# bigpon/QPNet

Measured on AMD Instinct MI355X. Metric: train steps/sec (batch-1 chunk-steps of RF+20000 samples, aggregate over GPUs), higher is better.
Workload: dtype f32; 1 GPU; config[1]: paper-size SI-QPNet (C=64,S=256,4F+4A) training step, forward+CE+backward+Adam on one chunk of 20900 samples (RF 946 + batch_length 19954), batch 1 per GPU; global_batch=1, parallelism=dp1 (utterance-sharded chunks, one flat-gradient all-reduce per step), backend=none, world_size=1, aux_1x1=frame rate (hoisted: K = 128 + one 4-deep step)

## Files before the change

qpnet_amd/csrc/train_bwd.hip:

```cpp
#include "train_common.h"
#include "train_post.h"
#include "qpn_handle.h"
#include <string.h>
#include <stdlib.h>
#include <math.h>

template <int MT>
__global__ __launch_bounds__(512) void k_post_bwd(TrainParams p, TrainBwd bw) {
    constexpr int TM = 16 * MT;
    extern __shared__ float sm[];
    const int S = p.S, Q = p.Q, LC = p.LC;
    const int ldp = tr_lda(Q > S ? Q : S), ldr = tr_lda(S);
    float* P = sm; float* R = sm + TM * ldp;
    const int b = blockIdx.y, t0 = blockIdx.x * TM;
    const int tid = threadIdx.x, lane = tid & 63, wave = tid >> 6;
    const int NTS = S / 16;
    const int npairs = (NTS + 1) / 2;
    const int np0 = wave < npairs ? wave : 0;
    const int pnt[2] = {2 * np0, (2 * np0 + 1 < NTS) ? 2 * np0 + 1 : 2 * np0};
    float my[2][MT][4], ms[2][MT][4];
    auto mask_load = [&](const float* src, float (&m)[2][MT][4]) {
#pragma unroll
        for (int j = 0; j < 2; ++j)
#pragma unroll
// ... 932 lines not shown
            for (int l = 0; l < w.nlayers; ++l) { sub.goff[l] = w.goff[l] + m0 * w.ldc; if (w.gbias[l] >= 0) sub.gbias[l] = w.gbias[l] + m0; }
            sub.ncol_groups = wgrad_col_groups(sub.M, sub.N);
            ok = wgrad2_any(sub, nch, generic, stream);
        }
        return ok;
    }
    if (wgrad3_any(w, nch, generic, stream)) return true;
    switch (w.bmode) {
    case 4: return false;
    case 1: return wgrad2_mode<1>(w, nch, stream);
    case 2: return wgrad2_mode<2>(w, nch, stream);
    case 3: return wgrad2_mode<3>(w, nch, stream);
    default: return wgrad2_mode<0>(w, nch, stream);
    }
}

__global__ void k_reduce_grad_s(const float* __restrict__ slab, const int* __restrict__ gdst, const int* __restrict__ gdst_list, const int* __restrict__ gzero, int n_gzero,
                                int nch, int gstage, int64_t n, float* __restrict__ g, float scale, int append_scale, int s0, int s1, int skip0, int skip1, int tail,
                                const int* __restrict__ status, int flag_again) {
    int64_t i = (int64_t)blockIdx.x * blockDim.x + threadIdx.x + s0;
    if (flag_again && append_scale && i == s0) g[n + 1] = (status && *status) ? 1.f : 0.f;
    if (i < s1) {
        if (i >= skip0 && i < skip1) return;
        const int k0 = gdst[i], k1 = gdst[i + 1];
        if (k0 == k1) return;
        float a = 0.f;
        const float* sp = slab + i;
        int c = 0;
        for (; c + 8 <= nch; c += 8) {
            float v[8];
#pragma unroll
            for (int k = 0; k < 8; ++k) v[k] = sp[(size_t)(c + k) * gstage];
            a += ((v[0] + v[1]) + (v[2] + v[3])) + ((v[4] + v[5]) + (v[6] + v[7]));
        }
        for (; c < nch; ++c) a += sp[(size_t)c * gstage];
        a *= scale;
        for (int k = k0; k < k1; ++k) g[gdst_list[k]] = a;
        return;
    }
    if (!tail) return;
    const int64_t j = i - s1;
    if (j < n_gzero) g[gzero[j]] = 0.f;
    else if (append_scale && j < n_gzero + 4 && !(flag_again && j == n_gzero + 1)) g[n + (j - n_gzero)] = j == n_gzero ? scale : (j == n_gzero + 1 && status && *status) ? 1.f : 0.f;
}

__global__ __launch_bounds__(256) void k_causal_bwd(TrainParams p, TrainBwd bw, int rows_per_wg, int CB) {
    extern __shared__ float tab[];
    const int C = p.C, Q = p.Q;
    const int tid = threadIdx.x;
    const int64_t total = (int64_t)p.B * p.N1;
    const int64_t r0 = (int64_t)blockIdx.x * rows_per_wg, r1 = r0 + rows_per_wg < total ? r0 + rows_per_wg : total;
    for (int cb = 0; cb < C; cb += CB) {
        const int cbv = C - cb < CB ? C - cb : CB;
        for (int i = tid; i < 2 * Q * CB; i += 256) tab[i] = 0.f;
        __syncthreads();
        const int cpr = cbv;
        for (int64_t idx = r0 * cpr + tid; idx < r1 * cpr; idx += 256) {
            const int64_t rr = idx / cpr; const int c = (int)(idx - rr * cpr);
            const int b = (int)(rr / p.N1), n = (int)(rr - (int64_t)b * p.N1);
            const size_t o = ((size_t)b * p.N1 + n) * C + cb + c;
            const float v = bw.DXA[0][o] + bw.DXB[0][o];
            const int64_t xo = (int64_t)p.T - p.N0 + n;
            int64_t s0 = p.x[(size_t)b * p.T + xo] % Q, s1 = p.x[(size_t)b * p.T + xo + 1] % Q;
            if (s0 < 0) s0 += Q;
            if (s1 < 0) s1 += Q;
            atomicAdd(&tab[(0 * Q + s0) * CB + c], v);
            atomicAdd(&tab[(1 * Q + s1) * CB + c], v);
        }
        __syncthreads();
        for (int i = tid; i < 2 * Q * cbv; i += 256) {
            const int c = i / (2 * Q), qt = i - c * 2 * Q, q = qt >> 1, tp = qt & 1;
            const float v = tab[(tp * Q + q) * CB + c];
            if (v != 0.f) atomicAdd(&bw.gflat[p.causal_w + ((size_t)(cb + c) * Q + q) * 2 + tp], v * bw.gscale);
        }
        for (int c = tid; c < cbv; c += 256) {
            float s = 0.f;
            for (int q = 0; q < Q; ++q) s += tab[(0 * Q + q) * CB + c];
            atomicAdd(&bw.gflat[p.causal_b + cb + c], s * bw.gscale);
        }
        __syncthreads();
    }
}

__global__ __launch_bounds__(128) void k_up_bwd(UpArgs u) { up_bwd_body(u, blockIdx.x, blockIdx.y, threadIdx.x, 128); }

__global__ __launch_bounds__(128) void k_aux_tail(AuxArgs p) {
    __shared__ float hrow[1024];
    __shared__ float red[2];
    const AuxGeom& ag = p.g;
    const int C = p.C, A = p.A, L = p.L, tid = threadIdx.x;
    const int bx = blockIdx.x;
    float v = 0.f;
    const bool role_a = bx < L * A;
    if (role_a) {
        const int l = bx / A, a = bx - l * A, n = tid;
        const size_t wi = (n < C ? ag.auxS[l] + (size_t)n * A : ag.auxT[l] + (size_t)(n - C) * A) + a;
        const float va = p.flat[wi];
        float e = 0.f;
        {
            float ev[TR_EB_SLOTS];
#pragma unroll
            for (int k = 0; k < TR_EB_SLOTS; ++k) ev[k] = p.EB[(size_t)(l * TR_EB_SLOTS + k) * 2 * C + n];
#pragma unroll
            for (int k = 0; k < TR_EB_SLOTS; ++k) e += ev[k];
        }
        float acc = 0.f;
        for (int b = 0; b < p.B; ++b) {
            const float* hb = p.h + ((size_t)b * A + a) * p.F + p.ffirst;
            const float* D = p.DPA + (size_t)(l * p.B + b) * (p.nfr + 1) * 2 * C + n;
            for (int f0 = 0; f0 < p.nfr; f0 += 1024) {
                const int nf = p.nfr - f0 < 1024 ? p.nfr - f0 : 1024;
                __syncthreads();
                for (int i = tid; i < nf; i += 128) hrow[i] = hb[f0 + i];
                __syncthreads();
                int f = 0;
                for (; f + 64 <= nf; f += 64) {
                    float d[64];
#pragma unroll
                    for (int k = 0; k < 64; ++k) d[k] = D[(size_t)(f0 + f + k) * 2 * C];
#pragma unroll
                    for (int k = 0; k < 64; ++k) acc += d[k] * hrow[f + k];
                }
                for (; f + 16 <= nf; f += 16) {
                    float d[16];
#pragma unroll
                    for (int k = 0; k < 16; ++k) d[k] = D[(size_t)(f0 + f + k) * 2 * C];
#pragma unroll
                    for (int k = 0; k < 16; ++k) acc += d[k] * hrow[f + k];
                }
                for (; f < nf; ++f) acc += D[(size_t)(f0 + f) * 2 * C] * hrow[f];
            }
        }
        p.gflat[wi] = (acc + p.flat[p.up_b] * e) * p.gscale;
        v = va * e;
    } else {
        const int j = bx - L * A;
        const int q0 = p.F * p.U - p.N1;
        const int items = L * p.B * p.nfr;
        for (int it = tid; it < items; it += 128) {
            const int fx = it % p.nfr, lb = it / p.nfr, l = lb / p.B;
            const int n = (p.ffirst + fx) * p.U + j - q0;
            if (n >= ag.s_out[l] && n < p.N1) v += p.GW[(size_t)lb * p.N1 + n];
        }
    }
    for (int sft = 32; sft >= 1; sft >>= 1) v += __shfl_xor(v, sft);
    if ((tid & 63) == 0) red[tid >> 6] = v;
    __syncthreads();
    if (tid == 0) {
        if (role_a) atomicAdd(p.gflat + p.up_b, (red[0] + red[1]) * p.gscale);
        else p.gflat[p.up_w + (bx - L * A)] = (red[0] + red[1]) * p.gscale;
    }
}

struct AdamReports { int* h_status; double* h_loss; const double* d_loss; };
__device__ __forceinline__ float adam_update(float* __restrict__ w, float* __restrict__ m, float* __restrict__ v, int64_t i, float gi,
                                             float lr, float b1, float b2, float eps, float wd, float bc1, float bc2_sqrt) {
    if (wd != 0.f) gi += wd * w[i];
    const float mi = m[i] + (gi - m[i]) * (1.0f - b1);
    const float vi = v[i] * b2 + (1.0f - b2) * gi * gi;
    m[i] = mi; v[i] = vi;
    const float denom = sqrtf(vi) / bc2_sqrt + eps;
    const float wn = w[i] - (lr / bc1) * (mi / denom);
    w[i] = wn;
    return wn;
}
template <bool EMA>
// ... 278 lines not shown
            } else {
                ok = ok && wgrad2_any(w, nch_side_, gen, st);
                w.A = bw.DY0; w.lda = S; w.M = S; w.B1 = p.S0; w.goff[0] = sl.g_p1; w.gbias[0] = sl.g_bp1;
                ok = ok && wgrad2_any(w, nch_side_, gen, st);
            }
            qpn_prof_mark(PG_WGRAD_POST, st);
        }
    };
    auto build_w1 = [&]() {
        Wg2 w = wbase;
        w.A = bw.DZ; w.A2 = nullptr; w.A_lstride = (size_t)B * N1 * 2 * C; w.lda = 2 * C; w.M = 2 * C; w.rowsA = N1;
        w.bmode = 3; w.B1 = p.X; w.B2 = nullptr; w.B_lstride = nDX; w.ldb = C; w.N = p.Ktp; w.Nvalid = p.hoist ? 2 * C : 2 * C + p.Ap; w.rowsB = N1;
        w.nlayers = L; w.ldc = p.Ktp; w.ncol_groups = wgrad_col_groups(w.M, w.N);
        for (int l = 0; l < L; ++l) {
            const TrLayer& ly = p.layers[l];
            w.row0A[l] = w.row0B[l] = ly.s_out; w.R[l] = N1 - ly.s_out; w.goff[l] = sl.g_w1[l]; w.gbias[l] = sl.g_b1[l];
            w.tap_off[l] = ly.tap_off; w.dil[l] = ly.dilation;
        }
        return w;
    };
    auto build_wr = [&]() {
        Wg2 w = wbase;
        w.A = bw.DXA[0] + nDX; w.A2 = wr_summed ? nullptr : bw.DXB[0] + nDX; w.A_lstride = nDX; w.lda = C; w.M = C; w.rowsA = N1;
        w.bmode = 0; w.B1 = p.TH; w.B2 = nullptr; w.B_lstride = nDX; w.ldb = C; w.N = C; w.Nvalid = C; w.rowsB = N1; w.ldc = C;
        w.nlayers = L; w.ncol_groups = wgrad_col_groups(w.M, w.N);
        for (int l = 0; l < L; ++l) {
            w.row0A[l] = w.row0B[l] = p.layers[l].s_out;
            w.R[l] = l == L - 1 ? 0 : N1 - p.layers[l].s_out; w.goff[l] = sl.g_wr[l]; w.gbias[l] = sl.g_br[l]; w.tap_off[l] = -1; w.dil[l] = 0;
        }
        return w;
    };
    const bool early_reduce = overlap && bw.gdst && sl.g_early1 > sl.g_early0 && k.reduce_early;
    const bool up_side = early_reduce && p.U > 0 && k.up_side;
    if (early_reduce) {
        nch_side_ = k.wgrad_chunks_side > 0 && k.wgrad_chunks_side <= nch ? k.wgrad_chunks_side : (nch <= 48 ? nch : 48);
    }
    if (overlap) {
        QPN_HIP(hipEventRecord(ev_fork, stream));
        QPN_HIP(hipStreamWaitEvent(side, ev_fork, 0));
        qpn_prof_mark(-1, side);
        launch_skip_post(side);
        if (early_reduce) { launch_reduce_early(bw, side, up_side ? 1 : 0, nch_side_); qpn_prof_mark(PG_GRAD_TAIL, side); }
        if (early_reduce && up_side && bw.ev_early && bw.early_recorded) { QPN_HIP(hipEventRecord(bw.ev_early, side)); *bw.early_recorded = 1; }
    }
    const int swz = k.xcd_swizzle ? 1 : 0;
    if (p.hoist && !persist) { qpn_set_error("internal: the frame-rate aux term needs the register-resident layer kernels"); return QPN_EINVAL; }
    if (stack_q) {
        const int rcq = qpn_launch_stack_bwd(p, bw, *sq, k, stream);
        if (rcq) return rcq;
    }
    for (int l = L - 1; l >= 0 && !stack_q; --l) {
        const TrLayer& ly = p.layers[l];
        const int rows = N1 - ly.s_out;
        const int tiles = (rows + 15) / 16;
        if (persist) {
            int G = qpn_num_cus() * 2; if (G > tiles) G = tiles;
            if (G > 1024) G = 1024;
            const size_t ldsp = (size_t)(8 * 16 * tr_lda(C) + 16 * tr_lda(2 * C) + 16 * tr_lda(p.Ktp) + 64) * sizeof(float);
            const bool last = l == L - 1;
            const void* kf = p.hoist ? (last ? (const void*)k_layer_bwd_p<8, true> : (const void*)k_layer_bwd_p<8, false>)
                                     : (last ? (const void*)k_layer_bwd_p<11, true> : (const void*)k_layer_bwd_p<11, false>);
            (void)hipFuncSetAttribute(kf, hipFuncAttributeMaxDynamicSharedMemorySize, (int)ldsp);
            if (p.hoist) {
                if (last) hipLaunchKernelGGL((k_layer_bwd_p<8, true>), dim3(G, B), dim3(256), ldsp, stream, p, bw, l, swz ? 2 : 0, tiles, p.scratch_rows);
                else hipLaunchKernelGGL((k_layer_bwd_p<8, false>), dim3(G, B), dim3(256), ldsp, stream, p, bw, l, swz ? 2 : 0, tiles, p.scratch_rows);
            } else {
                if (last) hipLaunchKernelGGL((k_layer_bwd_p<11, true>), dim3(G, B), dim3(256), ldsp, stream, p, bw, l, swz ? 2 : 0, tiles, p.scratch_rows);
                else hipLaunchKernelGGL((k_layer_bwd_p<11, false>), dim3(G, B), dim3(256), ldsp, stream, p, bw, l, swz ? 2 : 0, tiles, p.scratch_rows);
            }
        } else {
            if (lds_layer > 48 * 1024) (void)hipFuncSetAttribute((const void*)k_layer_bwd<1>, hipFuncAttributeMaxDynamicSharedMemorySize, (int)lds_layer);
            hipLaunchKernelGGL((k_layer_bwd<1>), dim3(tiles, B), dim3(256), lds_layer, stream, p, bw, l, l == L - 1 ? 1 : 0, swz);
        }
    }
    auto build_causal = [&]() {
        Wg2 w = wbase;
        w.nlayers = 2; w.ncol_groups = Q / (Q % 64 == 0 ? 64 : 128);      w.bmode = 4; w.xc = p.XC; w.B1 = w.B2 = nullptr; w.B_lstride = 0;
        w.A = bw.DXA[0]; w.A2 = bw.DXB[0]; w.A_lstride = 0; w.lda = C; w.M = C; w.rowsA = N1;
        w.N = Q; w.Nvalid = Q; w.rowsB = N1 + 1; w.ldb = 0; w.ldc = Q;
        for (int tp = 0; tp < 2; ++tp) { w.row0A[tp] = 0; w.row0B[tp] = tp; w.R[tp] = N1; w.goff[tp] = sl.g_cw + tp * C * Q; w.gbias[tp] = tp == 0 ? sl.g_cb : -1; w.tap_off[tp] = -1; w.dil[tp] = 0; }
        return w;
    };
    const bool wr_side = overlap && k.wr_side;
    if (wr_side || up_side) {
        QPN_HIP(hipEventRecord(bw.ev_mid, stream));
        QPN_HIP(hipStreamWaitEvent(side, bw.ev_mid, 0));
        qpn_prof_mark(-1, side);
        if (up_side) { if (p.hoist) launch_aux_tail(p, bw, ag, side); else launch_up_bwd(p, bw, side); qpn_prof_mark(PG_GRAD_TAIL, side); }
        if (wr_side) { ok = ok && wgrad2_any(build_wr(), nch, gen, side); qpn_prof_mark(PG_WGRAD_WR, side); }
    }
    if (overlap) QPN_HIP(hipEventRecord(ev_join, side));
    qpn_prof_mark(PG_LAYER_BWD, stream);
    ok = ok && wgrad2_any(build_w1(), nch, gen, stream);
    qpn_prof_mark(PG_WGRAD, stream);
    if (!wr_side) { ok = ok && wgrad2_any(build_wr(), nch, gen, stream); qpn_prof_mark(PG_WGRAD_WR, stream); }
    if (!overlap) launch_skip_post(stream);
    if (sl.g_cw >= 0) ok = ok && wgrad2_any(build_causal(), nch, gen, stream);
    qpn_prof_mark(PG_WGRAD_CAUSAL, stream);
    if (overlap) { QPN_HIP(hipStreamWaitEvent(stream, ev_join, 0)); qpn_prof_mark(-1, stream); }
    if (!ok) { qpn_set_error("weight-gradient tiles: unsupported geometry (n_resch <= 128 on this path; wider stacks take the GEMM path)"); return QPN_EINVAL; }
    return qpn_launch_grad_tail(p, bw, &ag, stream, early_reduce, up_side);
}

int qpn_launch_adam(float* w, const float* g, float* m, float* v, int64_t n, int step, float lr, float b1, float b2, float eps, float wd, const float* den, int* status,
                    int* h_status, double* h_loss, const double* d_loss, float* e, float omd, hipStream_t stream) {
    const double bc1 = 1.0 - pow((double)b1, step), bc2 = 1.0 - pow((double)b2, step);
    AdamReports rep; rep.h_status = status ? h_status : nullptr; rep.h_loss = d_loss ? h_loss : nullptr; rep.d_loss = d_loss;
    if (e) hipLaunchKernelGGL(k_adam_ema, dim3((unsigned)((n + 255) / 256)), dim3(256), 0, stream, w, g, m, v, n, lr, b1, b2, eps, wd, (float)bc1, (float)sqrt(bc2), den, status, rep, e, omd);
    else hipLaunchKernelGGL(k_adam, dim3((unsigned)((n + 255) / 256)), dim3(256), 0, stream, w, g, m, v, n, lr, b1, b2, eps, wd, (float)bc1, (float)sqrt(bc2), den, status, rep);
    qpn_prof_mark(PG_ADAM, stream);
    QPN_HIP(hipGetLastError());
    return QPN_OK;
}

int qpn_launch_adam_clip(float* w, const float* g, float* m, float* v, int64_t n, int step, float lr, float b1, float b2, float eps, float wd, const float* den, int* status,
                         int* h_status, double* h_loss, const double* d_loss, float max_norm, double* part, double* d_norm, double* h_norm, float* e, float omd, hipStream_t stream) {
    const double bc1 = 1.0 - pow((double)b1, step), bc2 = 1.0 - pow((double)b2, step);
    AdamReports rep; rep.h_status = status ? h_status : nullptr; rep.h_loss = d_loss ? h_loss : nullptr; rep.d_loss = d_loss;
    const int64_t want = ((n >> 2) + 1 + 255) / 256;
    const int nb = want < TR_GN_BLOCKS ? (int)want : TR_GN_BLOCKS;
    hipLaunchKernelGGL(k_grad_sumsq, dim3(nb), dim3(256), 0, stream, g, n, part);
    if (e) hipLaunchKernelGGL(k_adam_clip_ema, dim3((unsigned)((n + 255) / 256)), dim3(256), 0, stream, w, g, m, v, n, lr, b1, b2, eps, wd, (float)bc1, (float)sqrt(bc2), den, status, rep,
                              (const double*)part, nb, max_norm, d_norm, h_norm, e, omd);
    else hipLaunchKernelGGL(k_adam_clip, dim3((unsigned)((n + 255) / 256)), dim3(256), 0, stream, w, g, m, v, n, lr, b1, b2, eps, wd, (float)bc1, (float)sqrt(bc2), den, status, rep,
                            (const double*)part, nb, max_norm, d_norm, h_norm);
    qpn_prof_mark(PG_ADAM, stream);
    QPN_HIP(hipGetLastError());
    return QPN_OK;
}

int qpn_launch_grad_accum(float* acc, const float* g, int64_t cnt, int first, const int* status, int* h_status, double* h_loss, const double* d_loss, hipStream_t stream) {
    AdamReports rep; rep.h_status = status ? h_status : nullptr; rep.h_loss = d_loss ? h_loss : nullptr; rep.d_loss = d_loss;
    const int64_t want = ((cnt >> 2) + 1 + 255) / 256, cap = (int64_t)qpn_num_cus() * 8;
    const int nb = (int)(want < cap ? want : cap);
    hipLaunchKernelGGL(k_grad_accum, dim3(nb), dim3(256), 0, stream, acc, g, cnt, first ? 1 : 0, status, rep);
    qpn_prof_mark(PG_ADAM, stream);
    QPN_HIP(hipGetLastError());
    return QPN_OK;
}
```

qpnet_amd/csrc/train_common.h:

```cpp
#pragma once
#include "qpn_common.h"

typedef float f32x4 __attribute__((ext_vector_type(4)));

#define TR_MAXL QPN_MAX_LAYERS

__host__ __device__ static inline int tr_lda(int K) { return ((K + 29) / 32) * 32 + 2; }
__host__ __device__ static inline int tr_ldt(int N) { return ((N + 15) / 32) * 32 + 16; }

struct TrLayer {
    int adaptive, dilation;
    int s_in, s_out;
    int tap_off;
    int w1_f4, wr_f4;
    int w1t_f4, wrt_f4;
    int bias1, biasr;
};

struct TrainParams {
    int C, S, Q, A, Ap, L, U;
    int B, T, F, Td, BL, N1, N0, maxd;
    int Kt, Ktp;
    int LC;
    const float* flat;
// ... 6 lines not shown
    float* HUP;
    int hoist;
    int nfr, ffirst;
    float* PA;
    float2* WJ;
    int* TAP;
    int* XC;
    float* S0; float* Y0;
    float* logits;
    const int64_t* ce_tgt; int64_t ce_stride; float* ce_dlogits; double* ce_loss;
    int* status;
    float* scratch_rows;
    unsigned* qctl;
    int4* qtab;
    int4* qtab_b;
    int qtotal;
    int qP[TR_MAXL + 1];
    int qT[TR_MAXL];
    int ws_f4, p1_f4, p2_f4;
    int wst_f4, p1t_f4, p2t_f4;
    int bias_s, bias_p1, bias_p2;
    int64_t causal_w, causal_b, up_w, up_b;
    TrLayer layers[TR_MAXL];
};

struct TrainSlabs {
    int g_w1[TR_MAXL], g_b1[TR_MAXL], g_wr[TR_MAXL], g_br[TR_MAXL], g_ws[TR_MAXL], g_bs;
    int g_p1, g_bp1, g_p2, g_bp2;
    int g_early0, g_early1;
    int g_cw, g_cb;
};

struct TrainBwd {
    const float* dlogits; float* gflat;
    float* DXA[2]; float* DXB[2];
    float* DZ;
    float* DS0; float* DY0;
    float* DGS;
    float* DHUP;
    float* DPA;
    float* GW;
    float* EB;
    float* slab;
    const int* gdst; const int* gdst_list;
    const int* gzero; int n_gzero;
    int nch, gstage;
    int64_t n_params;
    const struct TrainSlabs* sl;
    float gscale;
    int append_scale;
    const int* status;
    hipStream_t side; hipEvent_t ev_fork, ev_join, ev_mid;
    hipEvent_t ev_early; int* early_recorded;
};


struct AuxGeom { int auxS[TR_MAXL], auxT[TR_MAXL], bias1[TR_MAXL], s_out[TR_MAXL]; };
struct AuxArgs {
    const float* flat; const float* h; float* PA; float* bp; const float* DPA; const float* EB; const float* GW; float* gflat;
    float gscale; int C, A, L, B, F, U, N1, nfr, ffirst; int64_t up_w, up_b;
    AuxGeom g;
};
static inline AuxArgs tr_aux_args(const TrainParams& p, const TrainBwd* bw, const AuxGeom& ag) {
    AuxArgs a; a.flat = p.flat; a.h = p.h; a.PA = p.PA; a.bp = p.bp; a.DPA = bw ? bw->DPA : nullptr; a.EB = bw ? bw->EB : nullptr; a.GW = bw ? bw->GW : nullptr;
    a.gflat = bw ? bw->gflat : nullptr; a.gscale = bw ? bw->gscale : 1.f;
    a.C = p.C; a.A = p.A; a.L = p.L; a.B = p.B; a.F = p.F; a.U = p.U; a.N1 = p.N1; a.nfr = p.nfr; a.ffirst = p.ffirst; a.up_w = p.up_w; a.up_b = p.up_b; a.g = ag;
    return a;
}
struct RefreshArgs { const int* wmap; float* wout; int64_t nw; const int* bstart; const int* blist; int nb; double* loss; };
struct TrainKnobs {
    bool serial;
    bool stack_q_fwd, stack_q_bwd;
    int stack_wgs, stack_wgs_bwd;
    bool persist_fwd, persist_bwd;
    bool wgrad_generic;
    int wgrad_chunks, wgrad_chunks_side;
    bool post_fuse;
    bool up_side, reduce_early, wr_side;
    bool post_pair, zero_in_post, post_wide;
    bool xcd_swizzle;
    bool ce_separate;
    bool event_fence;
    bool prep_fuse;
    bool aux_hoist;
    bool test_stack_gives_up;
};
void qpn_train_knobs_parse(TrainKnobs& k);

#define TR_QHEAD_STRIDE 1056
#define TR_QHDR_WORDS 17920
struct StackQ {
    unsigned* flags;
    unsigned* head;
    unsigned* stats;
    unsigned* abort;
    const int4* tab;
    unsigned epoch;
    unsigned epoch_pub;
    unsigned spin_limit;
    int total, nq;
};

__host__ __device__ __forceinline__ int tr_pa_off(const TrainParams& p, int l, int b, int n0) {
    const int q = p.F * p.U - p.N1 + n0;
    return ((l * p.B + b) * (p.nfr + 1) + (q / p.U - p.ffirst)) * 2 * p.C;
}

__device__ __forceinline__ void tr_queue_entry_fwd(const TrainParams& p, int pos, int4& a, int4& b) {
    const bool valid = pos < p.qtotal;
    const int ps = valid ? pos : 0;
    int l = 0;
    for (int k = 1; k < p.L; ++k) l += ps >= p.qP[k] ? 1 : 0;
    const int r = ps - p.qP[l], T = p.qT[l];
    const int bi = r / T, t = r - bi * T;
    const TrLayer ly = p.layers[l];
    const int n0 = ly.s_out + 16 * t;
    int first = 0, n = 0;
    if (valid && l > 0) {
        const int reach = ly.s_out - ly.s_in, s_prev = p.layers[l - 1].s_out;
        int lo = n0 - reach; if (lo < s_prev) lo = s_prev;
        int hi = n0 + 15; if (hi > p.N1 - 1) hi = p.N1 - 1;
        const int t_lo = (lo - s_prev) >> 4, t_hi = (hi - s_prev) >> 4;
        first = p.qP[l - 1] + bi * p.qT[l - 1] + t_lo; n = t_hi - t_lo + 1;
    }
    a = make_int4(n0, l | (bi << 8) | (l == p.L - 1 ? 1 << 24 : 0) | (valid ? 1 << 25 : 0), first, n);
    b = make_int4((l * p.B + bi) * p.N1, ly.tap_off + bi * p.N1, p.hoist ? tr_pa_off(p, l, bi, n0) : bi * p.N1, 0);
}

__device__ __forceinline__ void tr_queue_entry_bwd(const TrainParams& p, int pos, int4& a, int4& b) {
    const bool valid = pos < p.qtotal;
    const int ps = valid ? pos : 0;
    int k = 0, base = 0;
    for (int j = 0; j + 1 < p.L; ++j) { const int n = p.B * p.qT[p.L - 1 - j]; if (ps >= base + n) { base += n; k = j + 1; } else break; }
    const int l = p.L - 1 - k;
    const int r = ps - base, T = p.qT[l];
    const int bi = r / T, t = r - bi * T;
    const TrLayer ly = p.layers[l];
    const int n0 = ly.s_out + 16 * t;
    int first = 0, n = 0;
    if (valid && l < p.L - 1) {
        const TrLayer up = p.layers[l + 1];
        const int reach = up.s_out - up.s_in;
        int lo = n0 - up.s_out; if (lo < 0) lo = 0;
        int hi = n0 + 15 + reach; if (hi > p.N1 - 1) hi = p.N1 - 1;
        hi -= up.s_out;
        const int t_lo = lo >> 4, t_hi = hi >> 4;
        const int pbase = base - p.B * p.qT[l + 1];
        first = pbase + bi * p.qT[l + 1] + t_lo; n = t_hi - t_lo + 1;
    }
    a = make_int4(n0, l | (bi << 8) | (l == p.L - 1 ? 1 << 24 : 0) | (valid ? 1 << 25 : 0) | (ly.adaptive ? 1 << 26 : 0), first, n);
    b = make_int4((l * p.B + bi) * p.N1, ly.tap_off + bi * p.N1, p.hoist ? tr_pa_off(p, l, bi, n0) : bi * p.N1, bi * p.BL * p.LC + l * p.C);
}

struct TrainGemm {
    const float* wp;
    float* G;
    int K1;
    int N1g, Cg, Sg, Qg, LCg, Ktg;
    long w1[TR_MAXL], w1t[TR_MAXL], wr[TR_MAXL], wrt[TR_MAXL];
    long ws, wst, p1, p1t, p2, p2t;
};

#define TR_LDS_BARRIER() asm volatile("s_waitcnt lgkmcnt(0)\n\ts_barrier" ::: "memory")

int qpn_num_cus();

// ... 203 lines not shown
```

qpnet_amd/csrc/train_host.hip:

```cpp
#include "train_common.h"
#include "qpn_handle.h"
#include <algorithm>
#include <string.h>

int qpn_launch_fwd(const TrainParams& p, const TrainKnobs& k, const AuxGeom& ag, const StackQ* sq, hipStream_t stream, const TrainBwd* fuse_post_bwd, const RefreshArgs* rf);
bool qpn_step_prep_fits(const TrainParams& p);
void qpn_stack_fill(TrainParams& p);
int qpn_launch_ce(const float* logits, const int64_t* tgt, int64_t tgt_stride, int B, int BL, int Q, float* dlogits, double* loss, int* status, bool loss_cleared, hipStream_t stream);
int qpn_launch_bwd(const TrainParams& p, const TrainBwd& bw, const TrainKnobs& k, const AuxGeom& ag, const StackQ* sq, hipStream_t stream, bool post_done);
int qpn_launch_fwd_gemm(const TrainParams& p, const TrainGemm& w, hipStream_t stream);
int qpn_launch_bwd_gemm(const TrainParams& p, const TrainBwd& bw, const TrainGemm& w, hipStream_t stream);
int qpn_launch_adam(float* w, const float* g, float* m, float* v, int64_t n, int step, float lr, float b1, float b2, float eps, float wd, const float* den, int* status,
                    int* h_status, double* h_loss, const double* d_loss, float* e, float omd, hipStream_t stream);
int qpn_launch_adam_clip(float* w, const float* g, float* m, float* v, int64_t n, int step, float lr, float b1, float b2, float eps, float wd, const float* den, int* status,
                         int* h_status, double* h_loss, const double* d_loss, float max_norm, double* part, double* d_norm, double* h_norm, float* e, float omd, hipStream_t stream);
int qpn_launch_grad_accum(float* acc, const float* g, int64_t cnt, int first, const int* status, int* h_status, double* h_loss, const double* d_loss, hipStream_t stream);

#define LOSS_SLOT 72

struct TrainState {
    std::vector<int> h_wmap;
    std::vector<int> h_bstart, h_blist;
    std::vector<int> h_gsrc;
    int* d_wmap; float* d_wp; int* d_bstart; int* d_blist; float* d_bp; int n_bias;
    int* d_gdst; int* d_gdst_list; int* d_gzero; int n_gzero;
    bool hoist;
    TrainParams tp;
    TrainBwd bw;
    TrainSlabs slabs;
    TrainKnobs knobs;
    AuxGeom ag;
    float* d_ws; size_t ws_cap;
    int* d_tap; size_t tap_cap;
    int* d_status; double* d_loss;
    hipStream_t last_stream;
    int* h_status_pinned; hipEvent_t ev_status[2]; bool status_pending[2]; int status_newest;
    double* h_loss_pinned; hipEvent_t ev_loss[2]; bool loss_pending[2]; int loss_newest;
    double* d_gnorm; bool gnorm_last;
    bool gnorm_slot[2];
    double gnorm_collected; bool gnorm_collected_valid;
    bool fwd_valid;
    bool loss_clear;
    bool use_gemm;
    int* d_ctmap; float* d_ct;
    std::vector<int> h_gmap; int* d_gmap; float* d_gwp;
    TrainGemm gm;
    int64_t generation;
    hipStream_t side; hipEvent_t ev_fork, ev_join, ev_mid;
    hipEvent_t ev_early; int early_recorded; int64_t early_first;
    int64_t bwd_generation;
    const float* post_bwd_dlogits;
    bool post_bwd_done;
    bool stack_disabled;
    unsigned* d_sq; size_t sq_pos_cap, sq_per_dir;
    StackQ sqf, sqb;
};

static int env_int(const char* name, int dflt) { const char* e = getenv(name); return (e && *e) ? atoi(e) : dflt; }
void qpn_train_knobs_parse(TrainKnobs& k) {
    k.serial = env_int("QPN_TRAIN_SERIAL", 0) != 0;
    k.stack_q_fwd = env_int("QPN_STACK_QUEUE", 1) != 0;
    k.stack_q_bwd = k.stack_q_fwd && env_int("QPN_STACK_QUEUE_BWD", 1) != 0;
    k.stack_wgs = env_int("QPN_STACK_WGS", 0); if (k.stack_wgs < 0 || k.stack_wgs > 4096) k.stack_wgs = 0;
    k.stack_wgs_bwd = env_int("QPN_STACK_WGS_BWD", 0); if (k.stack_wgs_bwd < 0 || k.stack_wgs_bwd > 4096) k.stack_wgs_bwd = 0;
    k.persist_fwd = env_int("QPN_LAYER_PERSIST", 1) != 0;
    k.persist_bwd = env_int("QPN_LAYER_BWD_PERSIST", 1) != 0;
    k.wgrad_generic = getenv("QPN_WGRAD_GENERIC") != nullptr;
    k.wgrad_chunks = env_int("QPN_WGRAD_CHUNKS", 0); if (k.wgrad_chunks < 1 || k.wgrad_chunks > 512) k.wgrad_chunks = 0;
    k.wgrad_chunks_side = env_int("QPN_WGRAD_CHUNKS_SIDE", 0); if (k.wgrad_chunks_side < 1 || k.wgrad_chunks_side > 512) k.wgrad_chunks_side = 0;
    k.up_side = env_int("QPN_UP_SIDE", 1) != 0;
    k.reduce_early = env_int("QPN_REDUCE_EARLY", 1) != 0;
    k.wr_side = env_int("QPN_WR_SIDE", 1) != 0;
    k.post_fuse = env_int("QPN_POST_FUSE", 1) != 0;
    k.post_pair = env_int("QPN_POST_WGRAD_PAIR", 1) != 0;
    k.zero_in_post = env_int("QPN_ZERO_IN_POST", 1) != 0;
    k.post_wide = env_int("QPN_POST_WIDE", 1) != 0;
    k.xcd_swizzle = getenv("QPN_NO_XCD_SWIZZLE") == nullptr;
    k.ce_separate = getenv("QPN_CE_SEPARATE") != nullptr;
    k.event_fence = env_int("QPN_EVENT_FENCE", 0) == 1;
    k.aux_hoist = env_int("QPN_AUX_HOIST", 1) != 0;
    k.prep_fuse = env_int("QPN_PREP_FUSE", 1) != 0;
    k.test_stack_gives_up = false;
#ifdef QPN_TESTING
    k.test_stack_gives_up = env_int("QPN_TEST_STACK_GIVES_UP", 0) == 1;
#endif
}

int qpn_num_cus() {
    static int cached[64] = {0};
    int dev = 0;
    if (hipGetDevice(&dev) != hipSuccess || dev < 0 || dev >= 64) return 256;
    if (!cached[dev]) { int n = 0; if (hipDeviceGetAttribute(&n, hipDeviceAttributeMultiprocessorCount, dev) != hipSuccess || n < 1) n = 256; cached[dev] = n; }
    return cached[dev];
}

struct Prof { bool on = false; bool overlapped = false; std::vector<hipEvent_t> ev; std::vector<int> grp; std::vector<hipStream_t> st; size_t used = 0; };
static thread_local Prof g_prof;
bool qpn_prof_active() { return g_prof.on; }
bool qpn_prof_serial() { return g_prof.on && !g_prof.overlapped; }
void qpn_prof_mark(int group, hipStream_t stream) {
    Prof& P = g_prof;
    if (!P.on) return;
    if (P.used == P.ev.size()) { hipEvent_t e; if (hipEventCreate(&e) != hipSuccess) return; P.ev.push_back(e); P.grp.push_back(0); P.st.push_back(nullptr); }
    P.grp[P.used] = group; P.st[P.used] = stream;
    (void)hipEventRecord(P.ev[P.used++], stream);
}
extern "C" int qpn_train_profile_begin(qpn_handle* h, void* stream) {
    (void)h; g_prof.on = true; g_prof.overlapped = false; g_prof.used = 0;
    qpn_prof_mark(-1, (hipStream_t)stream);
    return QPN_OK;
}
extern "C" int qpn_train_profile_begin_overlapped(qpn_handle* h, void* stream) {
    (void)h; g_prof.on = true; g_prof.overlapped = true; g_prof.used = 0;
    qpn_prof_mark(-1, (hipStream_t)stream);
    return QPN_OK;
}
extern "C" int qpn_train_profile_mark(qpn_handle* h, int group, void* stream) {
    (void)h; qpn_prof_mark(group, (hipStream_t)stream); return QPN_OK;
}
extern "C" int qpn_train_profile_end(qpn_handle* h, float* h_ms, int n, void* stream) {
    Prof& P = g_prof;
    QPN_HIP(hipStreamSynchronize((hipStream_t)stream));
    if (h && h->train && h->train->side) QPN_HIP(hipStreamSynchronize(h->train->side));
    for (int i = 0; i < n; ++i) h_ms[i] = 0.f;
    for (size_t i = 1; i < P.used; ++i) {
        if (P.grp[i] < 0 || P.grp[i] >= n) continue;
        size_t j = i;
        while (j > 0 && P.st[j - 1] != P.st[i]) --j;
        if (j == 0) continue;
        float ms = 0.f;
        QPN_HIP(hipEventElapsedTime(&ms, P.ev[j - 1], P.ev[i]));
        h_ms[P.grp[i]] += ms;
    }
    P.on = false;
    return QPN_OK;
}

__global__ void k_gather_f(const float* __restrict__ flat, const int* __restrict__ map, float* __restrict__ out, int64_t n) {
    int64_t i = (int64_t)blockIdx.x * blockDim.x + threadIdx.x;
    if (i < n) { int m = map[i]; out[i] = m >= 0 ? flat[m] : 0.0f; }
}
__global__ void k_refresh(const float* __restrict__ flat, const int* __restrict__ wmap, float* __restrict__ wout, int64_t nw,
                          const int* __restrict__ ctmap, float* __restrict__ ct, int64_t nct,
                          const int* __restrict__ bstart, const int* __restrict__ blist, float* __restrict__ bp, int nb,
                          int* __restrict__ status, double* __restrict__ loss) {
    int64_t i = (int64_t)blockIdx.x * blockDim.x + threadIdx.x;
    if (i < nw) { const int m = wmap[i]; wout[i] = m >= 0 ? flat[m] : 0.0f; return; }
    i -= nw;
    if (i < nct) { ct[i] = flat[ctmap[i]]; return; }
    i -= nct;
    if (i < nb) { float a = 0.f; for (int j = bstart[i]; j < bstart[i + 1]; ++j) a += flat[blist[j]]; bp[i] = a; return; }
    i -= nb;
    (void)status;
    if (i >= 16 && i < 16 + 64) loss[i - 16] = 0.0;
}
template <class F>
static long kmajor_pack(std::vector<int>& map, int K, int Kp, int N, int Np, F src) {
    const long off = (long)map.size();
    map.resize(map.size() + (size_t)Kp * Np, -1);
    int* m = map.data() + off;
    for (int k = 0; k < K; ++k)
        for (int n = 0; n < N; ++n) m[(size_t)k * Np + n] = (int)src(k, n);
    return off;
// ... 781 lines not shown
```

Before: 1496 steps/s.

## Add sorted-row scatter kernel for causal conv weight gradient

Replaces the generic wgrad GEMM path for the causal (one-hot input) conv weight gradient with a dedicated kernel. Each block stages chunks of summed dX rows in LDS, ranks them by their quantized-input class, and segment-sums runs with equal class into a per-block LDS table, then writes the partial slab. Global row loads are double-buffered in registers. This exploits the one-hot sparsity instead of doing dense matmul work, at the cost of LDS pressure and a narrow geometry gate (C=64, Q 128/256).

```diff
diff --git a/qpnet_amd/csrc/train_bwd.hip b/qpnet_amd/csrc/train_bwd.hip
--- a/qpnet_amd/csrc/train_bwd.hip
+++ b/qpnet_amd/csrc/train_bwd.hip
@@ -1038,6 +1038,122 @@
     }
 }
 
+#define CR_RS 96
+#define CR_NT 512
+#define CR_NB 12
+static size_t causal_rows_lds(int Q) { return ((size_t)2 * Q * 65 + (size_t)CR_RS * 64 + 4 * CR_RS) * sizeof(float); }
+__global__ __launch_bounds__(CR_NT) void k_causal_rows(const float* __restrict__ A, const float* __restrict__ A2, const int* __restrict__ xc, float* __restrict__ slab,
+                                                       int gstage, int g_cw, int g_cb, int N1, int total, int nch, int Q) {
+    extern __shared__ float sm[];
+    constexpr int C = 64, LD = C + 1, RS = CR_RS, NL = RS * (C / 4) / CR_NT, SEG = RS / 4;
+    static_assert(RS * (C / 4) % CR_NT == 0 && 4 * RS <= CR_NT && RS % 8 == 0 && RS < 128 && CR_NT == 512, "a stage must tile the threads exactly; 7-bit row and rank fields");
+    float* tab = sm;
+    float* st = sm + (size_t)2 * Q * LD;
+    int* cls = (int*)(st + RS * C);
+    int* srt = cls + 2 * RS;
+    const int tid = threadIdx.x, lane = tid & 63, wave = tid >> 6, ch = blockIdx.x;
+    const int per = ((total + nch - 1) / nch + 31) / 32 * 32;
+    const int64_t rb64 = (int64_t)per * ch;
+    const int rbeg = rb64 < total ? (int)rb64 : total, rend = rb64 + per < total ? (int)(rb64 + per) : total;
+    for (int i = tid; i < 2 * Q * LD / 4; i += CR_NT) ((float4*)tab)[i] = make_float4(0.f, 0.f, 0.f, 0.f);
+    const int tp = wave & 1, sub = wave >> 1;
+    float* tb = tab + (size_t)tp * Q * LD + lane;
+    const int* so = srt + tp * RS;
+    float bsum = 0.f;
+    auto fetch = [&](int rs, float4 (&ra)[NL], float4 (&rb)[NL], int& rc) {
+#pragma unroll
+        for (int k = 0; k < NL; ++k) {
+            const int idx = tid + k * CR_NT;
+            int rr = rs + (idx >> 4); rr = rr < rend ? rr : rend - 1;
+            const size_t o = (size_t)rr * C + (idx & 15) * 4;
+            ra[k] = *(const float4*)(A + o);
+            rb[k] = *(const float4*)(A2 + o);
+        }
+        if (tid < 2 * RS) {
+            const int t = tid >= RS ? 1 : 0;
+            int rr = rs + tid - t * RS; rr = rr < rend ? rr : rend - 1;
+            rc = xc[rr + rr / N1 + t];
+        }
+    };
+    auto stage = [&](int rs, float4 (&ra)[NL], float4 (&rb)[NL], int& rc) {
+#pragma unroll
+        for (int k = 0; k < NL; ++k) {
+            const float4 a = ra[k], b = rb[k];
+            ((float4*)st)[tid + k * CR_NT] = make_float4(a.x + b.x, a.y + b.y, a.z + b.z, a.w + b.w);
+        }
+        if (tid < 2 * RS) { const int r = tid >= RS ? tid - RS : tid; cls[tid] = (((rs + r < rend && (unsigned)rc < (unsigned)Q) ? rc : Q) << 7) | r; }
+        __syncthreads();
+        if (rs + 2 * RS < rend) fetch(rs + 2 * RS, ra, rb, rc);
+        if (tid < 4 * RS) {
+            const int pr = tid >> 1, half = tid & 1, t = pr >= RS ? 1 : 0;
+            const int* cl = cls + t * RS;
+            const int key = cls[pr];
+            int rank = 0;
+#pragma unroll
+            for (int j = 0; j < RS / 2; j += 4) {
+                const int4 c4 = *(const int4*)(cl + half * (RS / 2) + j);
+                rank += (c4.x < key ? 1 : 0) + (c4.y < key ? 1 : 0) + (c4.z < key ? 1 : 0) + (c4.w < key ? 1 : 0);
+            }
+            rank += __shfl_xor(rank, 1);
+            if (half == 0) srt[t * RS + rank] = key;
+        }
+        __syncthreads();
+        {
+            const int k0 = so[lane], k0p = so[lane > 0 ? lane - 1 : 0], k1 = so[lane < RS - 64 ? 64 + lane : RS - 1], k1p = so[lane < RS - 64 ? 63 + lane : RS - 1];
+            const unsigned long long h0 = __ballot(lane == 0 || (k0 >> 7) != (k0p >> 7)), h1 = __ballot(lane < RS - 64 && (k1 >> 7) != (k1p >> 7));
+            const unsigned long long n0 = __ballot((k0 >> 7) >= Q), n1 = __ballot(lane < RS - 64 && (k1 >> 7) >= Q);
+            const int nv = n0 ? (int)__builtin_ctzll(n0) : n1 ? 64 + (int)__builtin_ctzll(n1) : RS;
+            auto bound = [&](int x) {
+                if (x < 64) { const unsigned long long m = h0 >> x; if (m) return x + (int)__builtin_ctzll(m); x = 64; }
+                if (x < RS) { const unsigned long long m = h1 >> (x - 64); if (m) return x + (int)__builtin_ctzll(m); }
+                return RS;
+            };
+            int a = bound(sub * SEG), b = bound(sub * SEG + SEG);
+            a = a < nv ? a : nv; b = b < nv ? b : nv;
+            for (int i0 = a; i0 < b; i0 += 64) {
+                const int ev = so[i0 + lane < RS ? i0 + lane : RS - 1];
+                const int n = b - i0 < 64 ? b - i0 : 64;
+                for (int i = 0; i < n; i += CR_NB) {
+                    int q[CR_NB]; float v[CR_NB], t[CR_NB];
+#pragma unroll
+                    for (int k = 0; k < CR_NB; ++k) {
+                        const bool ok = i + k < n;
+                        const int e = __builtin_amdgcn_readlane(ev, ok ? i + k : n - 1);
+                        q[k] = e >> 7;
+                        v[k] = st[(e & 127) * C + lane]; v[k] = ok ? v[k] : 0.f;
+                        t[k] = tb[q[k] * LD];
+                    }
+                    float sum = 0.f;
+#pragma unroll
+                    for (int k = 0; k < CR_NB; ++k) {
+                        sum = (k > 0 && q[k] == q[k - 1]) ? sum + v[k] : v[k];
+                        tb[q[k] * LD] = t[k] + sum;
+                        bsum += v[k];
+                    }
+                }
+            }
+        }
+        __syncthreads();
+    };
+    float4 ra0[NL], rb0[NL], ra1[NL], rb1[NL];
+    int rc0 = 0, rc1 = 0;
+    if (rbeg < rend) fetch(rbeg, ra0, rb0, rc0);
+    if (rbeg + RS < rend) fetch(rbeg + RS, ra1, rb1, rc1);
+    for (int rs = rbeg; rs < rend; rs += 2 * RS) {
+        stage(rs, ra0, rb0, rc0);
+        if (rs + RS < rend) stage(rs + RS, ra1, rb1, rc1);
+    }
+    if (tp == 0) st[sub * C + lane] = bsum;
+    __syncthreads();
+    float* out = slab + (size_t)ch * gstage;
+    const int qs = Q == 256 ? 8 : 7;
+    for (int i = tid; i < 2 * C * Q; i += CR_NT) {
+        const int q = i & (Q - 1), tc = i >> qs, c = tc & (C - 1), t = tc >> 6;
+        out[g_cw + i] = tab[((size_t)t * Q + q) * LD + c];
+    }
+    if (wave == 0) out[g_cb + lane] = ((st[lane] + st[C + lane]) + st[2 * C + lane]) + st[3 * C + lane];
+}
+
 __global__ __launch_bounds__(128) void k_up_bwd(UpArgs u) { up_bwd_body(u, blockIdx.x, blockIdx.y, threadIdx.x, 128); }
 
 __global__ __launch_bounds__(128) void k_aux_tail(AuxArgs p) {
@@ -1482,6 +1598,7 @@
         return w;
     };
     const bool wr_side = overlap && k.wr_side;
+    const bool causal_rows = k.causal_rows && sl.g_cw >= 0 && C == 64 && (Q == 128 || Q == 256) && (int64_t)B * N1 < (1ll << 31) - 2 * CR_RS;
     if (wr_side || up_side) {
         QPN_HIP(hipEventRecord(bw.ev_mid, stream));
         QPN_HIP(hipStreamWaitEvent(side, bw.ev_mid, 0));
@@ -1495,7 +1612,11 @@
     qpn_prof_mark(PG_WGRAD, stream);
     if (!wr_side) { ok = ok && wgrad2_any(build_wr(), nch, gen, stream); qpn_prof_mark(PG_WGRAD_WR, stream); }
     if (!overlap) launch_skip_post(stream);
-    if (sl.g_cw >= 0) ok = ok && wgrad2_any(build_causal(), nch, gen, stream);
+    if (causal_rows) {
+        const size_t lds_c = causal_rows_lds(Q);
+        (void)hipFuncSetAttribute((const void*)k_causal_rows, hipFuncAttributeMaxDynamicSharedMemorySize, (int)lds_c);
+        hipLaunchKernelGGL(k_causal_rows, dim3(nch), dim3(CR_NT), lds_c, stream, bw.DXA[0], bw.DXB[0], p.XC, bw.slab, bw.gstage, sl.g_cw, sl.g_cb, N1, B * N1, nch, Q);
+    } else if (sl.g_cw >= 0) ok = ok && wgrad2_any(build_causal(), nch, gen, stream);
     qpn_prof_mark(PG_WGRAD_CAUSAL, stream);
     if (overlap) { QPN_HIP(hipStreamWaitEvent(stream, ev_join, 0)); qpn_prof_mark(-1, stream); }
     if (!ok) { qpn_set_error("weight-gradient tiles: unsupported geometry (n_resch <= 128 on this path; wider stacks take the GEMM path)"); return QPN_EINVAL; }
diff --git a/qpnet_amd/csrc/train_common.h b/qpnet_amd/csrc/train_common.h
--- a/qpnet_amd/csrc/train_common.h
+++ b/qpnet_amd/csrc/train_common.h
@@ -112,6 +112,7 @@
     bool ce_separate;
     bool event_fence;
     bool prep_fuse;
+    bool causal_rows;
     bool aux_hoist;
     bool test_stack_gives_up;
 };
diff --git a/qpnet_amd/csrc/train_host.hip b/qpnet_amd/csrc/train_host.hip
--- a/qpnet_amd/csrc/train_host.hip
+++ b/qpnet_amd/csrc/train_host.hip
@@ -79,6 +79,7 @@
     k.ce_separate = getenv("QPN_CE_SEPARATE") != nullptr;
     k.event_fence = env_int("QPN_EVENT_FENCE", 0) == 1;
     k.aux_hoist = env_int("QPN_AUX_HOIST", 1) != 0;
+    k.causal_rows = env_int("QPN_CAUSAL_ROWS", 1) != 0;
     k.prep_fuse = env_int("QPN_PREP_FUSE", 1) != 0;
     k.test_stack_gives_up = false;
 #ifdef QPN_TESTING
```

After: 1507 steps/s (median of 6 runs). No clear change (+0.8%).
